# input-output-hk/plutus-halo2-verifier-gen

Measured on AMD Instinct MI355X. Metric: halo2_proofs_verified_per_sec, higher is better.
Workload: dtype u32

## Files before the change

### include/h2v.h

```cpp
#ifndef H2V_H
#define H2V_H
#include <stddef.h>
#include <stdint.h>
#ifdef __cplusplus
extern "C" {
#endif

#define H2V_OK 0
#define H2V_E_ARG (-1)
#define H2V_E_PLAN (-2)
#define H2V_E_DEVICE (-3)
#define H2V_E_LIMIT (-4)

#define H2V_MAX_MSM_TERMS 4096u

#define H2V_ST_BAD_SCALAR 1u
#define H2V_ST_INVERSE_OF_ZERO 2u
#define H2V_ST_SHORT_PROOF 4u
#define H2V_ST_BAD_POINT 8u
#define H2V_ST_PAIRING 16u
#define H2V_ST_RECURSION 32u

typedef struct h2v_plan h2v_plan;
typedef struct h2v_workspace h2v_workspace;
// ... 106 lines not shown
int h2v_plan_trace_slots(const h2v_plan *plan, uint32_t *slot_ids, uint32_t cap, uint32_t *n_out);
int h2v_trace(const h2v_plan *plan, const uint8_t *proof, size_t proof_len, const uint8_t *instances,
              const uint8_t *committed, uint8_t *scalars_out, uint8_t *msm_scalars_out ,
              uint8_t el_out[96], uint8_t er_out[96], uint32_t *status_out, uint8_t *accept_out);

int h2v_probe_field(int device, int op, uint32_t n, const uint32_t *a, const uint32_t *b, uint32_t *out);
int h2v_probe_blake2b(int device, uint32_t n, uint32_t len, const uint8_t *msgs, uint8_t *digests);
int h2v_probe_g1_decompress(int device, uint32_t n, const uint8_t *compressed, uint8_t *xy_be, uint8_t *valid);
int h2v_probe_g1_msm(int device, uint32_t n, uint32_t T, const uint8_t *scalars, const uint8_t *bases_compressed,
                     uint8_t *out_xy_be);
int h2v_probe_g1_msm_fixed(const h2v_plan *plan, uint32_t n, uint32_t bases_per_lane, const uint8_t *scalars, uint8_t *out_xy_be,
                           uint32_t *n_fix_out);
int h2v_probe_g1_msm_pippenger(int device, uint32_t n, const uint8_t *scalars, const uint8_t *bases_compressed,
                               uint8_t *out_xy_be);
int h2v_probe_quad_madd(int device, const uint32_t *pq, int neg, uint32_t *out);
int h2v_probe_pairing(const h2v_plan *plan, uint32_t n, const uint8_t *p1_compressed, const uint8_t *p2_compressed,
                      uint8_t *out);
int h2v_probe_pairing_ex(const h2v_plan *plan, uint32_t n, const uint8_t *p1_compressed, const uint8_t *p2_compressed,
                         uint8_t *out, int impl, uint8_t *dbg);

int h2v_shutdown(int device);

const char *h2v_last_error(void);
const char *h2v_build_id(void);
int h2v_device_count(void);

#ifdef __cplusplus
}
#endif
#endif
// ... 1 lines not shown
```

### plutus_halo2_verifier_gen_amd/backend.py

```python
from __future__ import annotations

import ctypes as C
import os
import sys
from typing import Optional

HERE = os.path.dirname(os.path.abspath(__file__))
LIB_PATH = os.path.join(HERE, "libh2v_hip.so")

H2V_OK = 0
ST_BAD_SCALAR, ST_INVERSE_OF_ZERO, ST_SHORT_PROOF, ST_BAD_POINT, ST_PAIRING, ST_RECURSION = 1, 2, 4, 8, 16, 32


class H2VError(RuntimeError):
    pass


class Batch(C.Structure):
    _fields_ = [("n", C.c_uint64), ("proofs", C.c_void_p), ("proof_off", C.c_void_p), ("instances", C.c_void_p),
                ("committed", C.c_void_p)]


class Timings(C.Structure):
    _fields_ = [("transcript_combiner_ms", C.c_float), ("g1_decompress_ms", C.c_float), ("g1_msm_ms", C.c_float),
# ... 38 lines not shown
    flags = RLC_ONE_STREAM if one_stream else 0
    if seed is None:
        return RlcOpts((C.c_uint8 * 32)(), flags)
    seed = bytes(seed)
    if len(seed) != 32:
        raise ValueError("the RLC seed is 32 bytes")
    return RlcOpts((C.c_uint8 * 32)(*seed), flags | RLC_SEED_GIVEN)


EXPORTS = [
    "h2v_plan_load", "h2v_plan_load_ex", "h2v_plan_free", "h2v_plan_info", "h2v_plan_compile", "h2v_blob_free", "h2v_workspace_create", "h2v_workspace_free",
    "h2v_workspace_timings", "h2v_workspace_hint_in_flight", "h2v_workspace_create_lanes", "h2v_workspace_create_multi", "h2v_workspace_defer_joins",
    "h2v_workspace_join", "h2v_workspace_lanes", "h2v_workspace_depth", "h2v_workspace_set_option", "h2v_workspace_get_option", "h2v_workspace_tune", "h2v_probe_set_option",
    "h2v_verify_batch", "h2v_verify_batch_submit", "h2v_verify_batch_wait", "h2v_verify_batch_device", "h2v_verify_batch_rlc", "h2v_verify_batch_rlc_device",
    "h2v_workspace_rlc_result", "h2v_probe_g1_msm_pippenger", "h2v_plan_trace_slots", "h2v_trace", "h2v_probe_field",
    "h2v_probe_blake2b", "h2v_probe_g1_decompress", "h2v_probe_g1_msm", "h2v_probe_g1_msm_fixed", "h2v_probe_quad_madd", "h2v_probe_pairing", "h2v_probe_pairing_ex",
    "h2v_last_error", "h2v_build_id",
    "h2v_device_count", "h2v_shutdown",
    "h2v_prepare_batch", "h2v_prepare_batch_device", "h2v_check_pairs", "h2v_check_pairs_device",
]

_lib = None


def lib():
    global _lib
    if _lib is None:
        if not os.path.exists(LIB_PATH):
            raise H2VError("HIP backend library %s is missing: run `python -c 'import __graft_entry__ as g; g.build()'` "
                           "(there is no CPU fallback)" % LIB_PATH)
        if "torch" not in sys.modules and os.environ.get("H2V_NO_TORCH_PRELOAD") is None:
# ... 26 lines not shown
        L.h2v_verify_batch.argtypes = [C.c_void_p, C.POINTER(Batch), C.c_void_p, C.c_void_p]
        L.h2v_verify_batch_device.argtypes = [C.c_void_p, C.POINTER(Batch), C.c_void_p, C.c_void_p, C.c_void_p,
                                              C.c_void_p, C.POINTER(Timings)]
        L.h2v_verify_batch_submit.argtypes = [C.c_void_p, C.POINTER(Batch), C.c_void_p, C.c_uint32, C.POINTER(RlcOpts)]
        L.h2v_verify_batch_wait.argtypes = [C.c_void_p, C.c_void_p, C.POINTER(C.c_int)]
        L.h2v_verify_batch_rlc.argtypes = [C.c_void_p, C.POINTER(Batch), C.c_void_p, C.c_void_p, C.POINTER(RlcOpts),
                                           C.POINTER(C.c_int)]
        L.h2v_verify_batch_rlc_device.argtypes = [C.c_void_p, C.POINTER(Batch), C.c_void_p, C.c_void_p, C.c_void_p,
                                                  C.c_void_p, C.POINTER(RlcOpts)]
        L.h2v_workspace_rlc_result.argtypes = [C.c_void_p, C.c_uint32, C.POINTER(C.c_uint32), C.POINTER(RlcTimings)]
        L.h2v_probe_g1_msm_pippenger.argtypes = [C.c_int, C.c_uint32, C.c_char_p, C.c_char_p, C.c_void_p]
        L.h2v_plan_trace_slots.argtypes = [C.c_void_p, C.POINTER(C.c_uint32), C.c_uint32, C.POINTER(C.c_uint32)]
        L.h2v_trace.argtypes = [C.c_void_p, C.c_char_p, C.c_size_t, C.c_char_p, C.c_char_p, C.c_void_p, C.c_void_p,
                                C.c_void_p, C.c_void_p, C.POINTER(C.c_uint32), C.POINTER(C.c_uint8)]
        L.h2v_probe_field.argtypes = [C.c_int, C.c_int, C.c_uint32, C.c_void_p, C.c_void_p, C.c_void_p]
        L.h2v_probe_blake2b.argtypes = [C.c_int, C.c_uint32, C.c_uint32, C.c_char_p, C.c_void_p]
        L.h2v_probe_g1_decompress.argtypes = [C.c_int, C.c_uint32, C.c_char_p, C.c_void_p, C.c_void_p]
        L.h2v_probe_g1_msm.argtypes = [C.c_int, C.c_uint32, C.c_uint32, C.c_char_p, C.c_char_p, C.c_void_p]
        L.h2v_probe_g1_msm_fixed.argtypes = [C.c_void_p, C.c_uint32, C.c_uint32, C.c_char_p, C.c_void_p, C.POINTER(C.c_uint32)]
        L.h2v_probe_pairing.argtypes = [C.c_void_p, C.c_uint32, C.c_char_p, C.c_char_p, C.c_void_p]
        L.h2v_probe_pairing_ex.argtypes = [C.c_void_p, C.c_uint32, C.c_char_p, C.c_char_p, C.c_void_p, C.c_int, C.c_void_p]
        L.h2v_shutdown.argtypes = [C.c_int]
        L.h2v_prepare_batch.argtypes = [C.c_void_p, C.POINTER(Batch), C.c_void_p, C.c_void_p, C.c_void_p]
        L.h2v_prepare_batch_device.argtypes = [C.c_void_p, C.POINTER(Batch), C.c_void_p, C.c_void_p, C.c_void_p, C.c_void_p]
        L.h2v_check_pairs.argtypes = [C.c_void_p, C.c_uint64, C.c_char_p, C.c_void_p, C.c_void_p, C.c_void_p]
        L.h2v_check_pairs_device.argtypes = [C.c_void_p, C.c_uint64, C.c_void_p, C.c_void_p, C.c_void_p, C.c_void_p, C.c_void_p]
        import atexit
        atexit.register(L.h2v_shutdown, -1)
        _lib = L
    return _lib
# ... 323 lines not shown


def probe_g1_msm_fixed(plan: DevicePlan, scalar_rows, bases_per_lane: int = 1):
    nf = C.c_uint32()
    if scalar_rows is None:
        lib().h2v_probe_g1_msm_fixed(plan.handle, 0, 1, None, None, C.byref(nf))
        return nf.value
    n = len(scalar_rows)
    sc = b"".join(int(s).to_bytes(32, "little") for row in scalar_rows for s in row)
    out = C.create_string_buffer(96 * n)
    check(lib().h2v_probe_g1_msm_fixed(plan.handle, n, bases_per_lane, sc, out, C.byref(nf)))
    assert all(len(row) == nf.value for row in scalar_rows)
    return [_unxy(out.raw[96 * i:96 * i + 96]) for i in range(n)]


def probe_quad_madd(p_xy, q_xy, neg: bool, device: int = 0):
    def limbs(v):
        return [(v >> (32 * i)) & 0xffffffff for i in range(12)]
    pq = (C.c_uint32 * 48)(*(limbs(p_xy[0]) + limbs(p_xy[1]) + limbs(q_xy[0]) + limbs(q_xy[1])))
    out = (C.c_uint32 * 210)()
    check(lib().h2v_probe_quad_madd(device, pq, 1 if neg else 0, out))
    from . import bls12_381 as bls
    rinv = pow(1 << 392, -1, bls.P)

    def val(o):
        return sum(out[o + k] << (28 * k) for k in range(14)) * rinv % bls.P
    return [(val(42 * j), val(42 * j + 14), val(42 * j + 28)) for j in range(5)]


def probe_g1_msm_pippenger(scalars, bases_compressed, device: int = 0):
# ... 26 lines not shown
```

### plutus_halo2_verifier_gen_amd/csrc/bls_consts.h

```cpp
#pragma once
#include <stdint.h>
#define H2V_DEVCONST static constexpr __device__ uint32_t
H2V_DEVCONST FP_MOD[12] = {0xffffaaabu, 0xb9feffffu, 0xb153ffffu, 0x1eabfffeu, 0xf6b0f624u, 0x6730d2a0u, 0xf38512bfu, 0x64774b84u, 0x434bacd7u, 0x4b1ba7b6u, 0x397fe69au, 0x1a0111eau};
static constexpr uint32_t FP_N0 = 0xfffcfffdu;
H2V_DEVCONST FP_ONE[12] = {0x0347fcb8u, 0x19d80000u, 0x6d2002b1u, 0x12e00cdeu, 0xa2090c72u, 0x37669f83u, 0xda0f73e0u, 0x09b09b42u, 0x8f1297bbu, 0xa7c515d9u, 0xfcfa012cu, 0x0577a659u};
H2V_DEVCONST FP_R2[12] = {0x510370edu, 0x626d1c34u, 0xc53e243du, 0xd65aec45u, 0x3317d3b1u, 0x4f36a009u, 0x5d74088bu, 0x8c10ea72u, 0x75865d11u, 0xd507320au, 0xa759fd5cu, 0x0c8d4cc8u};
H2V_DEVCONST FP_MOD28[14] = {0xfffaaabu, 0xfefffffu, 0x3ffffb9u, 0xfffeb15u, 0x6241eabu, 0xa0f6b0fu, 0xf6730d2u, 0xf38512bu, 0x4774b84u, 0x4bacd76u, 0xba7b643u, 0xe69a4b1u, 0x1ea397fu, 0x001a011u};
static constexpr uint32_t FP_N0_28 = 0xffcfffdu;
static constexpr uint32_t FP_FOLD_M = 0x9d83u;
H2V_DEVCONST FP_ONE28[14] = {0x347fcb8u, 0xd800000u, 0x2b119u, 0xcde6d2u, 0xc7212e0u, 0x83a2090u, 0x37669fu, 0xda0f73eu, 0x9b09b42u, 0x1297bb0u, 0x515d98fu, 0x12ca7cu, 0x659fcfau, 0x577au};
H2V_DEVCONST FP_C23P28[14] = {0xcda8c09u, 0x8faaaaau, 0x15720a4u, 0x893d93u, 0xfad6c24u, 0x8d68ebau, 0x54754b0u, 0x8d36a8du, 0x7f2d603u, 0xd0496f2u, 0x7467875u, 0xa2fbde3u, 0xf8a1126u, 0xc501u};
H2V_DEVCONST FP_C23N28[14] = {0x3251ea2u, 0x6f55555u, 0x2a8df15u, 0xf76ad82u, 0x676b287u, 0x138dc54u, 0xa1fdc22u, 0x664e69eu, 0xc847581u, 0x7b63683u, 0x4613dcdu, 0x439e6ceu, 0x2602859u, 0xdb0fu};
H2V_DEVCONST F28_KP[5][14] = {{0x0u, 0x0u, 0x0u, 0x0u, 0x0u, 0x0u, 0x0u, 0x0u, 0x0u, 0x0u, 0x0u, 0x0u, 0x0u, 0x0u}, {0xfffaaabu, 0xfefffffu, 0x3ffffb9u, 0xfffeb15u, 0x6241eabu, 0xa0f6b0fu, 0xf6730d2u, 0xf38512bu, 0x4774b84u, 0x4bacd76u, 0xba7b643u, 0xe69a4b1u, 0x1ea397fu, 0x1a011u}, {0xfff5556u, 0xfdfffffu, 0x7ffff73u, 0xfffd62au, 0xc483d57u, 0x41ed61eu, 0xece61a5u, 0xe70a257u, 0x8ee9709u, 0x9759aecu, 0x74f6c86u, 0xcd34963u, 0x3d472ffu, 0x34022u}, {0xfff0001u, 0xfcfffffu, 0xbffff2du, 0xfffc13fu, 0x26c5c03u, 0xe2e412eu, 0xe359277u, 0xda8f383u, 0xd65e28eu, 0xe306862u, 0x2f722c9u, 0xb3cee15u, 0x5beac7fu, 0x4e033u}, {0xffeaaacu, 0xfbfffffu, 0xffffee7u, 0xfffac54u, 0x8907aafu, 0x83dac3du, 0xd9cc34au, 0xce144afu, 0x1dd2e13u, 0x2eb35d9u, 0xe9ed90du, 0x9a692c6u, 0x7a8e5ffu, 0x68044u}};
H2V_DEVCONST F28_BIAS_3_1[14] = {0x2fff0001u, 0x2fcffffdu, 0x2bffff2bu, 0x2fffc13du, 0x226c5c01u, 0x2e2e412cu, 0x2e359275u, 0x2da8f381u, 0x2d65e28cu, 0x2e306860u, 0x22f722c7u, 0x2b3cee13u, 0x25beac7du, 0x4e031u};
H2V_DEVCONST F28_BIAS_5_2[14] = {0x3ffe5557u, 0x3faffffcu, 0x33fffe9eu, 0x3fff9767u, 0x3eb49958u, 0x324d1749u, 0x3d03f41au, 0x3c1995d8u, 0x36547995u, 0x37a6034cu, 0x3a468f4du, 0x38103775u, 0x39931f7cu, 0x82052u};
H2V_DEVCONST F28_BIAS_6_1[14] = {0x2ffe0002u, 0x2f9ffffdu, 0x27fffe59u, 0x2fff827du, 0x24d8b805u, 0x2c5c825au, 0x2c6b24edu, 0x2b51e705u, 0x2acbc51bu, 0x2c60d0c3u, 0x25ee4591u, 0x2679dc28u, 0x2b7d58fdu, 0x9c064u};
H2V_DEVCONST F28_BIAS_7_1[14] = {0x2ffdaaadu, 0x2f8ffffdu, 0x2bfffe13u, 0x2fff6d92u, 0x2afcd6b1u, 0x266bed69u, 0x2bd255c0u, 0x2a8a3831u, 0x2f4310a0u, 0x211b9e39u, 0x2195fbd5u, 0x24e380dau, 0x2d67927du, 0xb6075u};
H2V_DEVCONST F28_BIAS_11_1[14] = {0x2ffc5559u, 0x2f4ffffdu, 0x2bfffcfbu, 0x2fff19e7u, 0x238d5161u, 0x2ea999a7u, 0x296f190au, 0x276b7ce1u, 0x21203eb4u, 0x2406d413u, 0x2034d4e2u, 0x2e8a13a1u, 0x2510787cu, 0x11e0bau};
H2V_DEVCONST F28_BIAS_13_2[14] = {0x3ffbaaafu, 0x3f2ffffcu, 0x33fffc6eu, 0x3ffef011u, 0x3fd58eb8u, 0x32c86fc4u, 0x383d7aafu, 0x35dc1f38u, 0x3a0ed5bdu, 0x3d7c6efeu, 0x37844167u, 0x3b5d5d03u, 0x38e4eb7bu, 0x1520dbu};
H2V_DEVCONST F28_BIAS_17_8[14] = {0x9ffa555bu, 0x9eeffff6u, 0x93fffb50u, 0x9ffe9c60u, 0x98660962u, 0x9b061bfcu, 0x95da3df3u, 0x92bd63e2u, 0x9bec03cbu, 0x9067a4d1u, 0x96231a6fu, 0x9503efc4u, 0x908dd175u, 0x1ba11au};
H2V_DEVCONST F28_BIAS_20_1[14] = {0x2ff9555cu, 0x2ebffffdu, 0x2ffffa85u, 0x2ffe5da6u, 0x2ad2656du, 0x29345d31u, 0x240fd072u, 0x2066576du, 0x2951e661u, 0x2e980d3bu, 0x291a3d3fu, 0x2040dde0u, 0x264c7dfcu, 0x208154u};
H2V_DEVCONST F28_BIAS_21_1[14] = {0x2ff90007u, 0x2eaffffdu, 0x23fffa3fu, 0x2ffe48bcu, 0x20f68419u, 0x2343c841u, 0x23770145u, 0x2f9ea899u, 0x2dc931e5u, 0x2352dab1u, 0x24c1f383u, 0x2eaa8292u, 0x2836b77bu, 0x222165u};
H2V_DEVCONST F28_BIAS_29_2[14] = {0x3ff6555fu, 0x3e2ffffcu, 0x33fff80eu, 0x3ffda165u, 0x32177978u, 0x33bf20bbu, 0x3eb087d9u, 0x396131f7u, 0x31838e0cu, 0x39294663u, 0x31ffa59cu, 0x31f7a81fu, 0x3788837au, 0x2f21edu};
H2V_DEVCONST F28_BIAS_32_1[14] = {0x2ff55560u, 0x2dfffffdu, 0x2ffff73du, 0x2ffd62a5u, 0x2483d57du, 0x21ed61eau, 0x2ce61a52u, 0x270a257cu, 0x2ee9709cu, 0x2759aec6u, 0x24f6c867u, 0x2d349635u, 0x2d472ffau, 0x340221u};
H2V_DEVCONST FP_MOD30[13] = {0x3fffaaabu, 0x27fbffffu, 0x153ffffbu, 0x2affffacu, 0x30f6241eu, 0x34a83dau, 0x112bf673u, 0x12e13ce1u, 0x2cd76477u, 0x1ed90d2eu, 0x29a4b1bau, 0x3a8e5ff9u, 0x1a0111u};
static constexpr uint32_t FP_MINV30 = 0x30003u;
H2V_DEVCONST FP_R3[12] = {0xd1f7b890u, 0x22294cc4u, 0x56c9f3afu, 0xc0ccb5bau, 0xd975ccb5u, 0x89a8c5c0u, 0x6c968b4cu, 0x922672eau, 0xa691de8cu, 0x7c835652u, 0xbbb98497u, 0x141ab424u};
H2V_DEVCONST FR_MOD30[9] = {0x1u, 0x3ffffffcu, 0x3fe5bfefu, 0x2f6900bfu, 0x21d80553u, 0x27602026u, 0x17d48333u, 0x29d4ca67u, 0x73edu};
static constexpr uint32_t FR_MINV30 = 0x1u;
H2V_DEVCONST FP_B[12] = {0x0d1ff2e0u, 0x67600000u, 0xb4800ac4u, 0x4b803379u, 0x882431c8u, 0xdd9a7e0eu, 0x683dcf80u, 0x26c26d0bu, 0x3c4a5eecu, 0x9f145766u, 0xf3e804b2u, 0x15de9967u};
H2V_DEVCONST FP_TWO224[12] = {0x883cb548u, 0x5e8f53dbu, 0x0373eaf8u, 0xb9b546d2u, 0x1904502cu, 0x51b9fef6u, 0xe94c8520u, 0x8388341au, 0x58c0fea4u, 0x2865518au, 0x2cc4653du, 0x0a82ce35u};
H2V_DEVCONST FP_HALF_PLAIN[12] = {0xffffd555u, 0xdcff7fffu, 0x58a9ffffu, 0x0f55ffffu, 0x7b587b12u, 0xb3986950u, 0x79c2895fu, 0xb23ba5c2u, 0x21a5d66bu, 0x258dd3dbu, 0x1cbff34du, 0x0d0088f5u};
// ... 32 lines not shown
```

### plutus_halo2_verifier_gen_amd/csrc/h2v_capi.hip

```cpp
#include "../../include/h2v.h"

#include <hip/hip_runtime.h>
#include <stdio.h>
#include <stdlib.h>
#include <string.h>

#include <mutex>
#include <string>
#include <vector>

#include "h2v_kernels.hip"
#include "h2v_plancc.hpp"

static thread_local std::string g_err;
static int fail(int code, const std::string &msg) {
    g_err = msg;
    if (code == H2V_E_DEVICE && msg.find("hip: ") == std::string::npos) {
        const hipError_t e = hipPeekAtLastError();
        if (e != hipSuccess) g_err += std::string(" [hip: ") + hipGetErrorString(e) + "]";
    }
    return code;
}
#define HIPCHK(expr)                                                                                     \
    do {                                                                                                 \
// ... 2550 lines not shown
    HIPCHK(hipMemcpy(out, dout.p, bytes, hipMemcpyDeviceToHost));
    return H2V_OK;
}
extern "C" int h2v_probe_quad_madd(int device, const uint32_t *pq , int neg, uint32_t *out ) {
    int rc = pick_device(device);
    if (rc) return rc;
    DevBuf din, dout;
    if (din.alloc(48 * 4) || dout.alloc(210 * 4)) return fail(H2V_E_DEVICE, "hipMalloc failed");
    HIPCHK(hipMemcpy(din.p, pq, 48 * 4, hipMemcpyHostToDevice));
    hipLaunchKernelGGL(k_probe_quad_madd, dim3(1), dim3(64), 0, nullptr, din.as<uint32_t>(), neg, dout.as<uint32_t>());
    HIPCHK(hipGetLastError());
    HIPCHK(hipDeviceSynchronize());
    HIPCHK(hipMemcpy(out, dout.p, 210 * 4, hipMemcpyDeviceToHost));
    return H2V_OK;
}
extern "C" int h2v_probe_blake2b(int device, uint32_t n, uint32_t len, const uint8_t *msgs, uint8_t *digests) {
    int rc = pick_device(device);
    if (rc) return rc;
    if (!msgs || !digests || n == 0) return fail(H2V_E_ARG, "bad argument");
    DevBuf dm, dout;
    if (dm.alloc((size_t)n * len) || dout.alloc((size_t)n * 32)) return fail(H2V_E_DEVICE, "hipMalloc failed");
    if (len) HIPCHK(hipMemcpy(dm.p, msgs, (size_t)n * len, hipMemcpyHostToDevice));
    hipLaunchKernelGGL(k_probe_blake2b, dim3((n + 63) / 64), dim3(64), 0, nullptr, n, len, dm.as<uint8_t>(), dout.as<uint32_t>());
    HIPCHK(hipGetLastError());
    HIPCHK(hipDeviceSynchronize());
    HIPCHK(hipMemcpy(digests, dout.p, (size_t)n * 32, hipMemcpyDeviceToHost));
    return H2V_OK;
}
struct MiniPlan {
    H2vDevPlan d{};
// ... 151 lines not shown
```

### plutus_halo2_verifier_gen_amd/csrc/h2v_curve28.hpp

```cpp
#pragma once
#include "h2v_curve.hpp"
#include "h2v_fp28.hpp"

struct G1J28 { F28 x, y, z; };

H2V_DI void g1j28_from_affine(G1J28 &r, const G1A &a) {
    f28_from_fp(r.x, a.x);
    f28_from_fp(r.y, a.y);
    f28_set_one(r.z);
}
H2V_DI void g1j28_to_g1j(G1J &r, const G1J28 &p, const bool inf) {
    if (inf) { g1j_set_inf(r); return; }
    F28 z = p.z;
    f28_carry(z);
    f28_to_fp(r.x, p.x);
    f28_to_fp(r.y, p.y);
    f28_to_fp(r.z, z);
}
#define F28_MUL_(r, a, b) do { if (INL) f28_mul_inl(r, a, b); else f28_mul(r, a, b); } while (0)
#define F28_SQR_(r, a) do { if (INL) f28_sqr_inl(r, a); else f28_sqr(r, a); } while (0)
template <bool INL>
H2V_DI void g1j28_dbl_t(G1J28 &r, const G1J28 &p) {
    F28 X = p.x, Y = p.y, Z = p.z, A, B, C, D, t;
    F28_MUL_(Z, Y, Z); f28_mul_small<2>(Z, Z);
    F28_SQR_(A, X);
    F28_SQR_(B, Y);
    f28_add(t, X, B); F28_SQR_(t, t);
    F28_SQR_(C, B);
    f28_add(D, A, C);
    F28_SUB(t, t, D, 5, 2);
    f28_mul_small<2>(D, t); f28_carry(D);
    f28_mul_small<3>(A, A);
    F28_SQR_(X, A);
    f28_mul_small<2>(t, D);
    F28_SUB(X, X, t, 29, 2); f28_carry(X);
    F28_SUB(t, D, X, 32, 1);
    F28_MUL_(Y, A, t);
    f28_mul_small<8>(C, C);
    F28_SUB(Y, Y, C, 17, 8); f28_carry(Y);
    r.x = X; r.y = Y; r.z = Z;
}
#undef F28_MUL_
#undef F28_SQR_
H2V_DI void g1j28_dbl(G1J28 &r, const G1J28 &p) { g1j28_dbl_t<false>(r, p); }
H2V_DI int g1j28_add(G1J28 &r, const G1J28 &p, const G1J28 &q, const bool neg_q) {
    F28 X1 = p.x, Y1 = p.y, Z1 = p.z, a, b, c, t;
    f28_sqr(a, q.z);
    f28_mul(X1, X1, a);
    f28_mul(t, q.z, a); f28_mul(Y1, Y1, t);
    f28_sqr(a, Z1);
    f28_mul(b, q.x, a);
    f28_mul(t, Z1, a);
    {
        F28 qy = q.y, nq;
        F28_NEG(nq, qy, 20, 1);
        if (neg_q) qy = nq;
        f28_mul(c, qy, t);
    }
    F28_SUB(b, b, X1, 3, 1); f28_carry(b);
    F28_SUB(c, c, Y1, 3, 1); f28_carry(c);
    if (f28_is_zero_v5(b)) {
        if (f28_is_zero_v5(c)) { g1j28_dbl(r, p); return 1; }
        return 2;
    }
    f28_mul(Z1, Z1, q.z); f28_mul(Z1, Z1, b);
    f28_sqr(a, b);
    f28_mul(b, b, a);
    f28_mul(a, X1, a);
    f28_sqr(X1, c);
    F28_SUB(X1, X1, b, 3, 1);
    f28_mul_small<2>(t, a);
    F28_SUB(X1, X1, t, 5, 2); f28_carry(X1);
    F28_SUB(t, a, X1, 11, 1);
    f28_mul(c, c, t);
    f28_mul(t, Y1, b);
    F28_SUB(Y1, c, t, 3, 1); f28_carry(Y1);
    r.x = X1; r.y = Y1; r.z = Z1;
    return 0;
}
#define F28_MUL_(r, a, b) do { if (INL) f28_mul_inl(r, a, b); else f28_mul(r, a, b); } while (0)
#define F28_SQR_(r, a) do { if (INL) f28_sqr_inl(r, a); else f28_sqr(r, a); } while (0)
template <bool INL>
H2V_DI void g1j28_madd_ladder_t(G1J28 &r, const G1J28 &p, const F28 &qx, const F28 &qy_in, const bool neg_q) {
    F28 X1 = p.x, Y1 = p.y, Z1 = p.z, a, b, c, t;
    F28_SQR_(a, Z1);
    F28_MUL_(b, qx, a);
    F28_MUL_(t, Z1, a);
    {
        F28 qy = qy_in, nq;
        F28_NEG(nq, qy, 3, 1);
        if (neg_q) qy = nq;
        F28_MUL_(c, qy, t);
    }
    F28_SUB(b, b, X1, 32, 1);
    F28_SUB(c, c, Y1, 21, 1);
    F28_MUL_(Z1, Z1, b);
    F28_SQR_(a, b);
    F28_MUL_(b, b, a);
    F28_MUL_(a, X1, a);
    F28_SQR_(X1, c);
    F28_SUB(X1, X1, b, 3, 1);
    f28_mul_small<2>(t, a);
    F28_SUB(X1, X1, t, 5, 2); f28_carry(X1);
    F28_SUB(t, a, X1, 11, 1);
    F28_MUL_(c, c, t);
    F28_MUL_(t, Y1, b);
    F28_SUB(Y1, c, t, 3, 1); f28_carry(Y1);
    r.x = X1; r.y = Y1; r.z = Z1;
}
#undef F28_MUL_
#undef F28_SQR_
H2V_DI void g1j28_madd_ladder(G1J28 &r, const G1J28 &p, const F28 &qx, const F28 &qy_in, const bool neg_q) {
    g1j28_madd_ladder_t<false>(r, p, qx, qy_in, neg_q);
}
template <int LANE>
H2V_DI F28 f28_bcast(const F28 &a) {
    F28 r;
    constexpr int ctrl = LANE | (LANE << 2) | (LANE << 4) | (LANE << 6);
#pragma unroll
    for (int i = 0; i < 14; i++) {
        r.l[i] = (uint32_t)__builtin_amdgcn_update_dpp(0, (int)a.l[i], ctrl, 0xf, 0xf, false);
        asm volatile("" : "+v"(r.l[i]));
// ... 218 lines not shown
```

### plutus_halo2_verifier_gen_amd/csrc/h2v_field.hpp

```cpp
#pragma once
#include <hip/hip_runtime.h>
#include <stdint.h>
#include "bls_consts.h"

#define H2V_DI __device__ __forceinline__
#define H2V_DN __device__ __noinline__

template <int N>
struct Big {
    uint32_t v[N];
};
using Fp = Big<12>;
using Fr = Big<8>;

struct FpParams {
    static constexpr int N = 12;
    H2V_DI static uint32_t mod(int i) { return FP_MOD[i]; }
    H2V_DI static uint32_t one(int i) { return FP_ONE[i]; }
    H2V_DI static uint32_t r2(int i) { return FP_R2[i]; }
    static constexpr uint32_t n0 = FP_N0;
};
struct FrParams {
    static constexpr int N = 8;
    H2V_DI static uint32_t mod(int i) { return FR_MOD[i]; }
// ... 186 lines not shown
        acc += (uint64_t)m[k] * FP_MOD28[0];
        acc >>= 28;
    }
#pragma unroll
    for (int k = 14; k < 27; k++) {
#pragma unroll
        for (int i = k - 13; 2 * i < k; i++) acc += (uint64_t)d[i] * a[k - i];
        if ((k & 1) == 0) acc += (uint64_t)a[k / 2] * a[k / 2];
#pragma unroll
        for (int i = k - 13; i < 14; i++) acc += (uint64_t)m[i] * FP_MOD28[k - i];
        t[k - 14] = (uint32_t)acc & FP28_MASK;
        acc >>= 28;
    }
    t[13] = (uint32_t)acc;
}
H2V_DI Fp fp_mul_inl(const Fp &a, const Fp &b) {
    uint32_t a28[14], b28[14], t[14], w[12];
    fp_to28(a28, a);
    fp_to28(b28, b);
    fp_mont28(t, a28, b28);
    fp_from28(w, t);
    Fp r;
    FpF::cond_sub(r, w, 0);
    return r;
}
H2V_DI Fp fp_sqr_inl(const Fp &a) {
    uint32_t a28[14], t[14], w[12];
    fp_to28(a28, a);
    fp_montsqr28(t, a28);
    fp_from28(w, t);
// ... 117 lines not shown
```

### plutus_halo2_verifier_gen_amd/csrc/h2v_fp28.hpp

```cpp
#pragma once
#include "h2v_field.hpp"

struct F28 { uint32_t l[14]; };
typedef uint32_t u32x2 __attribute__((ext_vector_type(2)));
struct F28Regs { u32x4 a, b, c; u32x2 d; };

H2V_DI F28Regs f28_pack(const F28 &x) {
    F28Regs r;
    r.a = u32x4{x.l[0], x.l[1], x.l[2], x.l[3]};
    r.b = u32x4{x.l[4], x.l[5], x.l[6], x.l[7]};
    r.c = u32x4{x.l[8], x.l[9], x.l[10], x.l[11]};
    r.d = u32x2{x.l[12], x.l[13]};
    return r;
}
H2V_DI F28 f28_unpack(const u32x4 a, const u32x4 b, const u32x4 c, const u32x2 d) {
    F28 x;
    x.l[0] = a.x; x.l[1] = a.y; x.l[2] = a.z; x.l[3] = a.w;
    x.l[4] = b.x; x.l[5] = b.y; x.l[6] = b.z; x.l[7] = b.w;
    x.l[8] = c.x; x.l[9] = c.y; x.l[10] = c.z; x.l[11] = c.w;
    x.l[12] = d.x; x.l[13] = d.y;
    return x;
}
H2V_DN F28Regs f28_mul_raw(u32x4 a0, u32x4 a1, u32x4 a2, u32x2 a3, u32x4 b0, u32x4 b1, u32x4 b2, u32x2 b3) {
    const F28 a = f28_unpack(a0, a1, a2, a3), b = f28_unpack(b0, b1, b2, b3);
// ... 5 lines not shown
    const F28 a = f28_unpack(a0, a1, a2, a3);
    F28 t;
    fp_montsqr28(t.l, a.l);
    return f28_pack(t);
}
H2V_DI void f28_mul(F28 &r, const F28 &a, const F28 &b) {
    const F28Regs x = f28_pack(a), y = f28_pack(b);
    const F28Regs z = f28_mul_raw(x.a, x.b, x.c, x.d, y.a, y.b, y.c, y.d);
    r = f28_unpack(z.a, z.b, z.c, z.d);
}
H2V_DI void f28_sqr(F28 &r, const F28 &a) {
    const F28Regs x = f28_pack(a);
    const F28Regs z = f28_sqr_raw(x.a, x.b, x.c, x.d);
    r = f28_unpack(z.a, z.b, z.c, z.d);
}
H2V_DI void f28_mul_inl(F28 &r, const F28 &a, const F28 &b) { F28 t; fp_mont28(t.l, a.l, b.l); r = t; }
H2V_DI void f28_sqr_inl(F28 &r, const F28 &a) { F28 t; fp_montsqr28(t.l, a.l); r = t; }
H2V_DI void f28_add(F28 &r, const F28 &a, const F28 &b) {
#pragma unroll
    for (int i = 0; i < 14; i++) r.l[i] = a.l[i] + b.l[i];
}
template <int K>
H2V_DI void f28_mul_small(F28 &r, const F28 &a) {
#pragma unroll
    for (int i = 0; i < 14; i++) r.l[i] = a.l[i] * (uint32_t)K;
}
#define F28_SUB(r, a, b, K, M)                                                               \
    do {                                                                                     \
        _Pragma("unroll") for (int i_ = 0; i_ < 14; i_++)                                    \
            (r).l[i_] = (a).l[i_] + (F28_BIAS_##K##_##M[i_] - (b).l[i_]);                    \
// ... 98 lines not shown
```

### plutus_halo2_verifier_gen_amd/csrc/h2v_kernels.hip

```cpp
#include <hip/hip_runtime.h>
#include "h2v_curve28.hpp"
#include "h2v_plan.h"
#include "h2v_tower.hpp"
#include "h2v_pairing_coop.hpp"
#include "h2v_pairing_six.hpp"

__device__ static constexpr uint64_t B2_IV[8] = {
    0x6a09e667f3bcc908ull, 0xbb67ae8584caa73bull, 0x3c6ef372fe94f82bull, 0xa54ff53a5f1d36f1ull,
    0x510e527fade682d1ull, 0x9b05688c2b3e6c1full, 0x1f83d9abfb41bd6bull, 0x5be0cd19137e2179ull};
__device__ static constexpr uint8_t B2_SIGMA[12][16] = {
    {0, 1, 2, 3, 4, 5, 6, 7, 8, 9, 10, 11, 12, 13, 14, 15}, {14, 10, 4, 8, 9, 15, 13, 6, 1, 12, 0, 2, 11, 7, 5, 3},
    {11, 8, 12, 0, 5, 2, 15, 13, 10, 14, 3, 6, 7, 1, 9, 4}, {7, 9, 3, 1, 13, 12, 11, 14, 2, 6, 5, 10, 4, 0, 15, 8},
    {9, 0, 5, 7, 2, 4, 10, 15, 14, 1, 11, 12, 6, 8, 3, 13}, {2, 12, 6, 10, 0, 11, 8, 3, 4, 13, 7, 5, 15, 14, 1, 9},
    {12, 5, 1, 15, 14, 13, 4, 10, 0, 7, 6, 3, 9, 2, 8, 11}, {13, 11, 7, 14, 12, 1, 3, 9, 5, 0, 15, 4, 8, 6, 2, 10},
    {6, 15, 14, 9, 11, 3, 0, 8, 12, 2, 13, 7, 1, 4, 10, 5}, {10, 2, 8, 4, 7, 6, 1, 5, 15, 11, 9, 14, 3, 12, 13, 0},
    {0, 1, 2, 3, 4, 5, 6, 7, 8, 9, 10, 11, 12, 13, 14, 15}, {14, 10, 4, 8, 9, 15, 13, 6, 1, 12, 0, 2, 11, 7, 5, 3}};

H2V_DI uint64_t rotr64(uint64_t x, int n) { return (x >> n) | (x << (64 - n)); }

typedef __attribute__((address_space(3))) uint32_t h2v_lds_u32;
H2V_DN void b2_compress_lds(uint64_t (&h)[8], const uint32_t *msg_generic, uint64_t t, bool last) {
    const h2v_lds_u32 *msg = (const h2v_lds_u32 *)msg_generic;
    uint64_t v[16];
#pragma unroll
// ... 1333 lines not shown
    g1j28_from_affine(p1, P);
    g1j28_dbl(p2, p1);
    F28 qx, qy;
    f28_from_fp(qx, Q.x);
    f28_from_fp(qy, Q.y);
    g1j28_madd_ladder(a, p2, qx, qy, neg != 0);
    b = p2;
    g1j28_madd_quad(b, qx, qy, neg != 0);
    const int l = threadIdx.x;
    if (l == 0)
        for (int k = 0; k < 14; k++) { out[k] = a.x.l[k]; out[14 + k] = a.y.l[k]; out[28 + k] = a.z.l[k]; }
    if (l < 4)
        for (int k = 0; k < 14; k++) { out[42 * (1 + l) + k] = b.x.l[k]; out[42 * (1 + l) + 14 + k] = b.y.l[k]; out[42 * (1 + l) + 28 + k] = b.z.l[k]; }
}
extern "C" __global__ void __launch_bounds__(64)
k_probe_blake2b(uint32_t n, uint32_t len, const uint8_t *__restrict__ msgs, uint32_t *__restrict__ out) {
    __shared__ uint32_t sbuf[32 * 64];
    const int lane = threadIdx.x;
    const uint32_t i = blockIdx.x * 64 + lane;
    const uint32_t ii = i < n ? i : n - 1;
    Transcript tr;
    tr_init(tr);
    for (uint32_t k = 0; k < len; k++) tr_put(tr, sbuf, lane, msgs[(size_t)ii * len + k]);
    uint64_t h[4];
    tr_digest(tr, sbuf, lane, h);
    if (i < n) {
#pragma unroll
        for (int k = 0; k < 4; k++) { out[(size_t)i * 8 + 2 * k] = (uint32_t)h[k]; out[(size_t)i * 8 + 2 * k + 1] = (uint32_t)(h[k] >> 32); }
    }
}
// ... 29 lines not shown
```

Before: 1.252 million.

## Fuse sum-of-products Montgomery reductions in G1 doubling and addition formulas

```diff
diff --git a/include/h2v.h b/include/h2v.h
--- a/include/h2v.h
+++ b/include/h2v.h
@@ -144,6 +144,8 @@
 int h2v_probe_g1_msm_pippenger(int device, uint32_t n, const uint8_t *scalars, const uint8_t *bases_compressed,
                                uint8_t *out_xy_be);
 int h2v_probe_quad_madd(int device, const uint32_t *pq, int neg, uint32_t *out);
+int h2v_probe_f28_dot2(int device, int op, uint32_t n, const uint32_t *a, const uint32_t *b, const uint32_t *c, const uint32_t *d,
+                       uint32_t *out);
 int h2v_probe_pairing(const h2v_plan *plan, uint32_t n, const uint8_t *p1_compressed, const uint8_t *p2_compressed,
                       uint8_t *out);
 int h2v_probe_pairing_ex(const h2v_plan *plan, uint32_t n, const uint8_t *p1_compressed, const uint8_t *p2_compressed,
diff --git a/plutus_halo2_verifier_gen_amd/backend.py b/plutus_halo2_verifier_gen_amd/backend.py
--- a/plutus_halo2_verifier_gen_amd/backend.py
+++ b/plutus_halo2_verifier_gen_amd/backend.py
@@ -76,7 +76,7 @@
     "h2v_workspace_join", "h2v_workspace_lanes", "h2v_workspace_depth", "h2v_workspace_set_option", "h2v_workspace_get_option", "h2v_workspace_tune", "h2v_probe_set_option",
     "h2v_verify_batch", "h2v_verify_batch_submit", "h2v_verify_batch_wait", "h2v_verify_batch_device", "h2v_verify_batch_rlc", "h2v_verify_batch_rlc_device",
     "h2v_workspace_rlc_result", "h2v_probe_g1_msm_pippenger", "h2v_plan_trace_slots", "h2v_trace", "h2v_probe_field",
-    "h2v_probe_blake2b", "h2v_probe_g1_decompress", "h2v_probe_g1_msm", "h2v_probe_g1_msm_fixed", "h2v_probe_quad_madd", "h2v_probe_pairing", "h2v_probe_pairing_ex",
+    "h2v_probe_blake2b", "h2v_probe_g1_decompress", "h2v_probe_g1_msm", "h2v_probe_g1_msm_fixed", "h2v_probe_quad_madd", "h2v_probe_f28_dot2", "h2v_probe_pairing", "h2v_probe_pairing_ex",
     "h2v_last_error", "h2v_build_id",
     "h2v_device_count", "h2v_shutdown",
     "h2v_prepare_batch", "h2v_prepare_batch_device", "h2v_check_pairs", "h2v_check_pairs_device",
@@ -133,6 +133,7 @@
         L.h2v_trace.argtypes = [C.c_void_p, C.c_char_p, C.c_size_t, C.c_char_p, C.c_char_p, C.c_void_p, C.c_void_p,
                                 C.c_void_p, C.c_void_p, C.POINTER(C.c_uint32), C.POINTER(C.c_uint8)]
         L.h2v_probe_field.argtypes = [C.c_int, C.c_int, C.c_uint32, C.c_void_p, C.c_void_p, C.c_void_p]
+        L.h2v_probe_f28_dot2.argtypes = [C.c_int, C.c_int, C.c_uint32, C.c_void_p, C.c_void_p, C.c_void_p, C.c_void_p, C.c_void_p]
         L.h2v_probe_blake2b.argtypes = [C.c_int, C.c_uint32, C.c_uint32, C.c_char_p, C.c_void_p]
         L.h2v_probe_g1_decompress.argtypes = [C.c_int, C.c_uint32, C.c_char_p, C.c_void_p, C.c_void_p]
         L.h2v_probe_g1_msm.argtypes = [C.c_int, C.c_uint32, C.c_uint32, C.c_char_p, C.c_char_p, C.c_void_p]
@@ -486,6 +487,29 @@
     return [_unxy(out.raw[96 * i:96 * i + 96]) for i in range(n)]
 
 
+DOT2_MUL, DOT2_SQR, DOT2_SQR2, DOT2_DBL, DOT2_MADD, DOT2_ADD, DOT2_INLINE, DOT2_NEG_Q = 0, 1, 2, 8, 9, 10, 16, 64
+
+
+def probe_f28_dot2(op: int, a, b=None, c=None, d=None, device: int = 0):
+    n = len(a)
+    field = (op & 15) < 8
+
+    def pack(recs):
+        if recs is None:
+            return None
+        flat = [l for r in recs for l in (r if field else [x for rec in r for x in rec])]
+        assert len(flat) == n * (14 if field else 42)
+        return (C.c_uint32 * len(flat))(*flat)
+
+    out = (C.c_uint32 * (n * (14 if field else 44)))()
+    if field and b is None:
+        b = a
+    check(lib().h2v_probe_f28_dot2(device, op, n, pack(a), pack(b), pack(c), pack(d), out))
+    if field:
+        return [list(out[14 * i:14 * i + 14]) for i in range(n)]
+    return [(tuple(list(out[44 * i + 14 * j:44 * i + 14 * j + 14]) for j in range(3)), int(out[44 * i + 42])) for i in range(n)]
+
+
 def probe_quad_madd(p_xy, q_xy, neg: bool, device: int = 0):
     def limbs(v):
         return [(v >> (32 * i)) & 0xffffffff for i in range(12)]
diff --git a/plutus_halo2_verifier_gen_amd/csrc/bls_consts.h b/plutus_halo2_verifier_gen_amd/csrc/bls_consts.h
--- a/plutus_halo2_verifier_gen_amd/csrc/bls_consts.h
+++ b/plutus_halo2_verifier_gen_amd/csrc/bls_consts.h
@@ -16,6 +16,7 @@
 H2V_DEVCONST F28_BIAS_5_2[14] = {0x3ffe5557u, 0x3faffffcu, 0x33fffe9eu, 0x3fff9767u, 0x3eb49958u, 0x324d1749u, 0x3d03f41au, 0x3c1995d8u, 0x36547995u, 0x37a6034cu, 0x3a468f4du, 0x38103775u, 0x39931f7cu, 0x82052u};
 H2V_DEVCONST F28_BIAS_6_1[14] = {0x2ffe0002u, 0x2f9ffffdu, 0x27fffe59u, 0x2fff827du, 0x24d8b805u, 0x2c5c825au, 0x2c6b24edu, 0x2b51e705u, 0x2acbc51bu, 0x2c60d0c3u, 0x25ee4591u, 0x2679dc28u, 0x2b7d58fdu, 0x9c064u};
 H2V_DEVCONST F28_BIAS_7_1[14] = {0x2ffdaaadu, 0x2f8ffffdu, 0x2bfffe13u, 0x2fff6d92u, 0x2afcd6b1u, 0x266bed69u, 0x2bd255c0u, 0x2a8a3831u, 0x2f4310a0u, 0x211b9e39u, 0x2195fbd5u, 0x24e380dau, 0x2d67927du, 0xb6075u};
+H2V_DEVCONST F28_BIAS_9_4[14] = {0x5ffd0003u, 0x5f6ffffau, 0x53fffd84u, 0x5fff43bau, 0x57451406u, 0x5a8ac385u, 0x5aa0b762u, 0x58fada86u, 0x5831a7a7u, 0x5a913923u, 0x58e56858u, 0x51b6ca3au, 0x513c057au, 0xea095u};
 H2V_DEVCONST F28_BIAS_11_1[14] = {0x2ffc5559u, 0x2f4ffffdu, 0x2bfffcfbu, 0x2fff19e7u, 0x238d5161u, 0x2ea999a7u, 0x296f190au, 0x276b7ce1u, 0x21203eb4u, 0x2406d413u, 0x2034d4e2u, 0x2e8a13a1u, 0x2510787cu, 0x11e0bau};
 H2V_DEVCONST F28_BIAS_13_2[14] = {0x3ffbaaafu, 0x3f2ffffcu, 0x33fffc6eu, 0x3ffef011u, 0x3fd58eb8u, 0x32c86fc4u, 0x383d7aafu, 0x35dc1f38u, 0x3a0ed5bdu, 0x3d7c6efeu, 0x37844167u, 0x3b5d5d03u, 0x38e4eb7bu, 0x1520dbu};
 H2V_DEVCONST F28_BIAS_17_8[14] = {0x9ffa555bu, 0x9eeffff6u, 0x93fffb50u, 0x9ffe9c60u, 0x98660962u, 0x9b061bfcu, 0x95da3df3u, 0x92bd63e2u, 0x9bec03cbu, 0x9067a4d1u, 0x96231a6fu, 0x9503efc4u, 0x908dd175u, 0x1ba11au};
diff --git a/plutus_halo2_verifier_gen_amd/csrc/h2v_capi.hip b/plutus_halo2_verifier_gen_amd/csrc/h2v_capi.hip
--- a/plutus_halo2_verifier_gen_amd/csrc/h2v_capi.hip
+++ b/plutus_halo2_verifier_gen_amd/csrc/h2v_capi.hip
@@ -2588,6 +2588,30 @@
     HIPCHK(hipMemcpy(out, dout.p, 210 * 4, hipMemcpyDeviceToHost));
     return H2V_OK;
 }
+extern "C" int h2v_probe_f28_dot2(int device, int op, uint32_t n, const uint32_t *a, const uint32_t *b, const uint32_t *c, const uint32_t *d,
+                                  uint32_t *out) {
+    int rc = pick_device(device);
+    if (rc) return rc;
+    const int what = op & 15;
+    const bool field = what <= 2, point = what >= 8 && what <= 10;
+    if ((op & ~(15 | 16 | 64)) != 0 || !(field || point) || (what == 10 && (op & 16)) || n == 0 || !a || !out) return fail(H2V_E_ARG, "bad argument");
+    if (field ? (!b || !c || !d) : (what != 8 && !b)) return fail(H2V_E_ARG, "bad argument");
+    const size_t in_b = (size_t)n * (field ? 14 : 42) * 4, out_b = (size_t)n * (field ? 14 : 44) * 4;
+    DevBuf da, db, dc, dd, dout;
+    if (da.alloc(in_b) || db.alloc(in_b) || dc.alloc(in_b) || dd.alloc(in_b) || dout.alloc(out_b)) return fail(H2V_E_DEVICE, "hipMalloc failed");
+    HIPCHK(hipMemcpy(da.p, a, in_b, hipMemcpyHostToDevice));
+    if (field || what != 8) HIPCHK(hipMemcpy(db.p, b, in_b, hipMemcpyHostToDevice));
+    if (field) {
+        HIPCHK(hipMemcpy(dc.p, c, in_b, hipMemcpyHostToDevice));
+        HIPCHK(hipMemcpy(dd.p, d, in_b, hipMemcpyHostToDevice));
+    }
+    hipLaunchKernelGGL(k_probe_f28_dot2, dim3((n + 63) / 64), dim3(64), 0, nullptr, op, n, da.as<uint32_t>(), db.as<uint32_t>(),
+                       dc.as<uint32_t>(), dd.as<uint32_t>(), dout.as<uint32_t>());
+    HIPCHK(hipGetLastError());
+    HIPCHK(hipDeviceSynchronize());
+    HIPCHK(hipMemcpy(out, dout.p, out_b, hipMemcpyDeviceToHost));
+    return H2V_OK;
+}
 extern "C" int h2v_probe_blake2b(int device, uint32_t n, uint32_t len, const uint8_t *msgs, uint8_t *digests) {
     int rc = pick_device(device);
     if (rc) return rc;
diff --git a/plutus_halo2_verifier_gen_amd/csrc/h2v_curve28.hpp b/plutus_halo2_verifier_gen_amd/csrc/h2v_curve28.hpp
--- a/plutus_halo2_verifier_gen_amd/csrc/h2v_curve28.hpp
+++ b/plutus_halo2_verifier_gen_amd/csrc/h2v_curve28.hpp
@@ -21,23 +21,21 @@
 #define F28_SQR_(r, a) do { if (INL) f28_sqr_inl(r, a); else f28_sqr(r, a); } while (0)
 template <bool INL>
 H2V_DI void g1j28_dbl_t(G1J28 &r, const G1J28 &p) {
-    F28 X = p.x, Y = p.y, Z = p.z, A, B, C, D, t;
-    F28_MUL_(Z, Y, Z); f28_mul_small<2>(Z, Z);
+    F28 X = p.x, Y = p.y, Z = p.z, A, B, D, t;
+    F28_NEG(t, Y, 21, 1);
+    F28_MUL_(Z, t, Z); f28_mul_small<2>(Z, Z);
     F28_SQR_(A, X);
     F28_SQR_(B, Y);
-    f28_add(t, X, B); F28_SQR_(t, t);
-    F28_SQR_(C, B);
-    f28_add(D, A, C);
-    F28_SUB(t, t, D, 5, 2);
-    f28_mul_small<2>(D, t); f28_carry(D);
+    F28_MUL_(D, X, B);
     f28_mul_small<3>(A, A);
     F28_SQR_(X, A);
-    f28_mul_small<2>(t, D);
-    F28_SUB(X, X, t, 29, 2); f28_carry(X);
-    F28_SUB(t, D, X, 32, 1);
-    F28_MUL_(Y, A, t);
-    f28_mul_small<8>(C, C);
-    F28_SUB(Y, Y, C, 17, 8); f28_carry(Y);
+    f28_mul_small<8>(t, D);
+    F28_SUB(X, X, t, 17, 8); f28_carry(X);
+    f28_mul_small<4>(D, D);
+    F28_SUB(t, X, D, 9, 4); f28_carry(t);
+    f28_mul_small<2>(B, B);
+    if (INL) f28_dot2_sqr_inl<2>(Y, B, A, t);
+    else f28_dot2_sqr<2>(Y, B, A, t);
     r.x = X; r.y = Y; r.z = Z;
 }
 #undef F28_MUL_
@@ -58,23 +56,22 @@
         f28_mul(c, qy, t);
     }
     F28_SUB(b, b, X1, 3, 1); f28_carry(b);
-    F28_SUB(c, c, Y1, 3, 1); f28_carry(c);
+    F28_SUB(c, Y1, c, 3, 1); f28_carry(c);
     if (f28_is_zero_v5(b)) {
         if (f28_is_zero_v5(c)) { g1j28_dbl(r, p); return 1; }
         return 2;
     }
     f28_mul(Z1, Z1, q.z); f28_mul(Z1, Z1, b);
     f28_sqr(a, b);
-    f28_mul(b, b, a);
-    f28_mul(a, X1, a);
+    F28_NEG(t, a, 3, 1);
+    f28_mul(b, b, t);
+    f28_mul(a, X1, t);
     f28_sqr(X1, c);
-    F28_SUB(X1, X1, b, 3, 1);
+    f28_add(X1, X1, b);
     f28_mul_small<2>(t, a);
-    F28_SUB(X1, X1, t, 5, 2); f28_carry(X1);
-    F28_SUB(t, a, X1, 11, 1);
-    f28_mul(c, c, t);
-    f28_mul(t, Y1, b);
-    F28_SUB(Y1, c, t, 3, 1); f28_carry(Y1);
+    f28_add(X1, X1, t); f28_carry(X1);
+    f28_add(t, a, X1);
+    f28_dot2(Y1, c, t, Y1, b);
     r.x = X1; r.y = Y1; r.z = Z1;
     return 0;
 }
@@ -93,19 +90,19 @@
         F28_MUL_(c, qy, t);
     }
     F28_SUB(b, b, X1, 32, 1);
-    F28_SUB(c, c, Y1, 21, 1);
+    F28_SUB(c, Y1, c, 3, 1);
     F28_MUL_(Z1, Z1, b);
     F28_SQR_(a, b);
-    F28_MUL_(b, b, a);
-    F28_MUL_(a, X1, a);
+    F28_NEG(t, a, 3, 1);
+    F28_MUL_(b, b, t);
+    F28_MUL_(a, X1, t);
     F28_SQR_(X1, c);
-    F28_SUB(X1, X1, b, 3, 1);
+    f28_add(X1, X1, b);
     f28_mul_small<2>(t, a);
-    F28_SUB(X1, X1, t, 5, 2); f28_carry(X1);
-    F28_SUB(t, a, X1, 11, 1);
-    F28_MUL_(c, c, t);
-    F28_MUL_(t, Y1, b);
-    F28_SUB(Y1, c, t, 3, 1); f28_carry(Y1);
+    f28_add(X1, X1, t); f28_carry(X1);
+    f28_add(t, a, X1);
+    if (INL) f28_dot2_inl(Y1, c, t, Y1, b);
+    else f28_dot2(Y1, c, t, Y1, b);
     r.x = X1; r.y = Y1; r.z = Z1;
 }
 #undef F28_MUL_
diff --git a/plutus_halo2_verifier_gen_amd/csrc/h2v_field.hpp b/plutus_halo2_verifier_gen_amd/csrc/h2v_field.hpp
--- a/plutus_halo2_verifier_gen_amd/csrc/h2v_field.hpp
+++ b/plutus_halo2_verifier_gen_amd/csrc/h2v_field.hpp
@@ -224,6 +224,68 @@
     }
     t[13] = (uint32_t)acc;
 }
+H2V_DI void fp_mont28_dot2(uint32_t (&t)[14], const uint32_t (&a)[14], const uint32_t (&b)[14], const uint32_t (&c)[14],
+                           const uint32_t (&d)[14]) {
+    uint32_t m[14];
+    uint64_t acc = 0;
+#pragma unroll
+    for (int k = 0; k < 14; k++) {
+#pragma unroll
+        for (int i = 0; i <= k; i++) acc += (uint64_t)a[i] * b[k - i];
+#pragma unroll
+        for (int i = 0; i <= k; i++) acc += (uint64_t)c[i] * d[k - i];
+#pragma unroll
+        for (int i = 0; i < k; i++) acc += (uint64_t)m[i] * FP_MOD28[k - i];
+        m[k] = ((uint32_t)acc * FP_N0_28) & FP28_MASK;
+        acc += (uint64_t)m[k] * FP_MOD28[0];
+        acc >>= 28;
+    }
+#pragma unroll
+    for (int k = 14; k < 27; k++) {
+#pragma unroll
+        for (int i = k - 13; i < 14; i++) acc += (uint64_t)a[i] * b[k - i];
+#pragma unroll
+        for (int i = k - 13; i < 14; i++) acc += (uint64_t)c[i] * d[k - i];
+#pragma unroll
+        for (int i = k - 13; i < 14; i++) acc += (uint64_t)m[i] * FP_MOD28[k - i];
+        t[k - 14] = (uint32_t)acc & FP28_MASK;
+        acc >>= 28;
+    }
+    t[13] = (uint32_t)acc;
+}
+template <int W>
+H2V_DI void fp_mont28_dot2_sqr(uint32_t (&t)[14], const uint32_t (&a)[14], const uint32_t (&c)[14], const uint32_t (&d)[14]) {
+    uint32_t m[14], o[14];
+#pragma unroll
+    for (int i = 0; i < 14; i++) o[i] = a[i] * (uint32_t)(2 * W);
+    uint64_t acc = 0;
+#pragma unroll
+    for (int k = 0; k < 14; k++) {
+#pragma unroll
+        for (int i = 0; 2 * i < k; i++) acc += (uint64_t)o[i] * a[k - i];
+        if ((k & 1) == 0) acc += (uint64_t)(a[k / 2] * (uint32_t)W) * a[k / 2];
+#pragma unroll
+        for (int i = 0; i <= k; i++) acc += (uint64_t)c[i] * d[k - i];
+#pragma unroll
+        for (int i = 0; i < k; i++) acc += (uint64_t)m[i] * FP_MOD28[k - i];
+        m[k] = ((uint32_t)acc * FP_N0_28) & FP28_MASK;
+        acc += (uint64_t)m[k] * FP_MOD28[0];
+        acc >>= 28;
+    }
+#pragma unroll
+    for (int k = 14; k < 27; k++) {
+#pragma unroll
+        for (int i = k - 13; 2 * i < k; i++) acc += (uint64_t)o[i] * a[k - i];
+        if ((k & 1) == 0) acc += (uint64_t)(a[k / 2] * (uint32_t)W) * a[k / 2];
+#pragma unroll
+        for (int i = k - 13; i < 14; i++) acc += (uint64_t)c[i] * d[k - i];
+#pragma unroll
+        for (int i = k - 13; i < 14; i++) acc += (uint64_t)m[i] * FP_MOD28[k - i];
+        t[k - 14] = (uint32_t)acc & FP28_MASK;
+        acc >>= 28;
+    }
+    t[13] = (uint32_t)acc;
+}
 H2V_DI Fp fp_mul_inl(const Fp &a, const Fp &b) {
     uint32_t a28[14], b28[14], t[14], w[12];
     fp_to28(a28, a);
diff --git a/plutus_halo2_verifier_gen_amd/csrc/h2v_fp28.hpp b/plutus_halo2_verifier_gen_amd/csrc/h2v_fp28.hpp
--- a/plutus_halo2_verifier_gen_amd/csrc/h2v_fp28.hpp
+++ b/plutus_halo2_verifier_gen_amd/csrc/h2v_fp28.hpp
@@ -43,6 +43,35 @@
     const F28Regs z = f28_sqr_raw(x.a, x.b, x.c, x.d);
     r = f28_unpack(z.a, z.b, z.c, z.d);
 }
+H2V_DN F28Regs f28_dot2_raw(u32x4 a0, u32x4 a1, u32x4 a2, u32x2 a3, u32x4 b0, u32x4 b1, u32x4 b2, u32x2 b3,
+                            u32x4 c0, u32x4 c1, u32x4 c2, u32x2 c3, u32x4 d0, u32x4 d1, u32x4 d2, u32x2 d3) {
+    const F28 a = f28_unpack(a0, a1, a2, a3), b = f28_unpack(b0, b1, b2, b3), c = f28_unpack(c0, c1, c2, c3), d = f28_unpack(d0, d1, d2, d3);
+    F28 t;
+    fp_mont28_dot2(t.l, a.l, b.l, c.l, d.l);
+    return f28_pack(t);
+}
+H2V_DI void f28_dot2(F28 &r, const F28 &a, const F28 &b, const F28 &c, const F28 &d) {
+    const F28Regs x = f28_pack(a), y = f28_pack(b), u = f28_pack(c), v = f28_pack(d);
+    const F28Regs z = f28_dot2_raw(x.a, x.b, x.c, x.d, y.a, y.b, y.c, y.d, u.a, u.b, u.c, u.d, v.a, v.b, v.c, v.d);
+    r = f28_unpack(z.a, z.b, z.c, z.d);
+}
+template <int W>
+H2V_DN F28Regs f28_dot2_sqr_raw(u32x4 a0, u32x4 a1, u32x4 a2, u32x2 a3, u32x4 c0, u32x4 c1, u32x4 c2, u32x2 c3,
+                                u32x4 d0, u32x4 d1, u32x4 d2, u32x2 d3) {
+    const F28 a = f28_unpack(a0, a1, a2, a3), c = f28_unpack(c0, c1, c2, c3), d = f28_unpack(d0, d1, d2, d3);
+    F28 t;
+    fp_mont28_dot2_sqr<W>(t.l, a.l, c.l, d.l);
+    return f28_pack(t);
+}
+template <int W>
+H2V_DI void f28_dot2_sqr(F28 &r, const F28 &a, const F28 &c, const F28 &d) {
+    const F28Regs x = f28_pack(a), u = f28_pack(c), v = f28_pack(d);
+    const F28Regs z = f28_dot2_sqr_raw<W>(x.a, x.b, x.c, x.d, u.a, u.b, u.c, u.d, v.a, v.b, v.c, v.d);
+    r = f28_unpack(z.a, z.b, z.c, z.d);
+}
+H2V_DI void f28_dot2_inl(F28 &r, const F28 &a, const F28 &b, const F28 &c, const F28 &d) { F28 t; fp_mont28_dot2(t.l, a.l, b.l, c.l, d.l); r = t; }
+template <int W>
+H2V_DI void f28_dot2_sqr_inl(F28 &r, const F28 &a, const F28 &c, const F28 &d) { F28 t; fp_mont28_dot2_sqr<W>(t.l, a.l, c.l, d.l); r = t; }
 H2V_DI void f28_mul_inl(F28 &r, const F28 &a, const F28 &b) { F28 t; fp_mont28(t.l, a.l, b.l); r = t; }
 H2V_DI void f28_sqr_inl(F28 &r, const F28 &a) { F28 t; fp_montsqr28(t.l, a.l); r = t; }
 H2V_DI void f28_add(F28 &r, const F28 &a, const F28 &b) {
diff --git a/plutus_halo2_verifier_gen_amd/csrc/h2v_kernels.hip b/plutus_halo2_verifier_gen_amd/csrc/h2v_kernels.hip
--- a/plutus_halo2_verifier_gen_amd/csrc/h2v_kernels.hip
+++ b/plutus_halo2_verifier_gen_amd/csrc/h2v_kernels.hip
@@ -1371,6 +1371,41 @@
         for (int k = 0; k < 14; k++) { out[42 * (1 + l) + k] = b.x.l[k]; out[42 * (1 + l) + 14 + k] = b.y.l[k]; out[42 * (1 + l) + 28 + k] = b.z.l[k]; }
 }
 extern "C" __global__ void __launch_bounds__(64)
+k_probe_f28_dot2(int op, uint32_t n, const uint32_t *__restrict__ a, const uint32_t *__restrict__ b, const uint32_t *__restrict__ c,
+                 const uint32_t *__restrict__ d, uint32_t *__restrict__ out) {
+    const uint32_t i = blockIdx.x * 64 + threadIdx.x;
+    if (i >= n) return;
+    const int what = op & 15;
+    const bool inl = (op & 16) != 0, neg = (op & 64) != 0;
+    if (what < 8) {
+        F28 x, y, u, v, r;
+#pragma unroll
+        for (int k = 0; k < 14; k++) { x.l[k] = a[(size_t)i * 14 + k]; y.l[k] = b[(size_t)i * 14 + k]; u.l[k] = c[(size_t)i * 14 + k]; v.l[k] = d[(size_t)i * 14 + k]; }
+        if (what == 0) { if (inl) f28_dot2_inl(r, x, y, u, v); else f28_dot2(r, x, y, u, v); }
+        else if (what == 1) { if (inl) f28_dot2_sqr_inl<1>(r, x, u, v); else f28_dot2_sqr<1>(r, x, u, v); }
+        else { if (inl) f28_dot2_sqr_inl<2>(r, x, u, v); else f28_dot2_sqr<2>(r, x, u, v); }
+#pragma unroll
+        for (int k = 0; k < 14; k++) out[(size_t)i * 14 + k] = r.l[k];
+        return;
+    }
+    G1J28 P, Q, r;
+#pragma unroll
+    for (int k = 0; k < 14; k++) {
+        P.x.l[k] = a[(size_t)i * 42 + k]; P.y.l[k] = a[(size_t)i * 42 + 14 + k]; P.z.l[k] = a[(size_t)i * 42 + 28 + k];
+        Q.x.l[k] = what == 8 ? 0u : b[(size_t)i * 42 + k]; Q.y.l[k] = what == 8 ? 0u : b[(size_t)i * 42 + 14 + k];
+        Q.z.l[k] = what == 8 ? 0u : b[(size_t)i * 42 + 28 + k];
+    }
+    r = P;
+    int rc = 0;
+    if (what == 8) { if (inl) g1j28_dbl_t<true>(r, P); else g1j28_dbl_t<false>(r, P); }
+    else if (what == 9) { if (inl) g1j28_madd_ladder_t<true>(r, P, Q.x, Q.y, neg); else g1j28_madd_ladder_t<false>(r, P, Q.x, Q.y, neg); }
+    else rc = g1j28_add(r, P, Q, neg);
+#pragma unroll
+    for (int k = 0; k < 14; k++) { out[(size_t)i * 44 + k] = r.x.l[k]; out[(size_t)i * 44 + 14 + k] = r.y.l[k]; out[(size_t)i * 44 + 28 + k] = r.z.l[k]; }
+    out[(size_t)i * 44 + 42] = (uint32_t)rc;
+    out[(size_t)i * 44 + 43] = 0u;
+}
+extern "C" __global__ void __launch_bounds__(64)
 k_probe_blake2b(uint32_t n, uint32_t len, const uint8_t *__restrict__ msgs, uint32_t *__restrict__ out) {
     __shared__ uint32_t sbuf[32 * 64];
     const int lane = threadIdx.x;
```

Measured after the change: 1.282 million (median of 6 runs). 2.4% higher.
